# openai/Video-Pre-Training

Hardware: AMD Instinct MI355X
Metric: frames/sec (fwd) [+ bc_step.ms_per_step], 2x policy, 128x128x3 seq=128 (higher is better)
Workload: dtype bf16; 1 GPU; foundation-model-2x policy forward (IMPALA CNN + 4-layer banded transformer + heads), batch=64 seq=128 uint8 128x128x3 frames per GPU, KV memory carried, random-init weights; global_batch=64, seq_len=128, parallelism=dp1 replicas (no collective in forward; BC step: gradient all-reduce)

## Files before the change

### video-pre-training_amd/csrc/vpt_conv3x3.hip

```cpp
#include "vpt_common.h"
#include "vpt_kernels.h"
#include <stdlib.h>
#include <type_traits>
#ifndef VPT_EPI_NO_CLAMP_RELU
#define VPT_EPI_NO_CLAMP_RELU 0
#endif
#ifdef VPT_CONV_PROFILE
#define CONV_ABLATE (a.ablate)
#else
#define CONV_ABLATE 0
#endif
#if defined(VPT_CONV_PROFILE) && defined(VPT_CONV_FWD_ABLATE)
#define FWD_NO_DMA (VPT_CONV_FWD_ABLATE == 1 || VPT_CONV_FWD_ABLATE == 4)
#define FWD_NO_HALO (VPT_CONV_FWD_ABLATE == 2 || VPT_CONV_FWD_ABLATE == 4)
#else
#define FWD_NO_DMA 0
#define FWD_NO_HALO 0
#endif
#define A_RS 80
#define A_BYTES (324 * A_RS)
#define B_BYTES (3 * 128 * 64)
#define KK_OFF (A_BYTES + 2 * B_BYTES)
#define KK_BYTES (9 * 128 * 4)
#define BT_OFF (KK_OFF + KK_BYTES + 64)
#define SMEM_BYTES (BT_OFF + 512)
#define PT_RS 272
static_assert(256 * PT_RS <= KK_OFF, "the pooled mode's output tile must fit below the epilogue table");

__device__ __forceinline__ int sub_row(int i) { return ((i >> 4) ^ (i >> 2) ^ (i >> 3)) & 1; }

template <int U> __device__ __forceinline__ f32x4 ac_get(const f32x16& v) {
  return __builtin_shufflevector(v, v, 4 * U, 4 * U + 1, 4 * U + 2, 4 * U + 3);
}
template <int U> __device__ __forceinline__ void ac_set(f32x16& v, const f32x4 c) {
  const f32x16 w = __builtin_shufflevector(c, c, 0, 1, 2, 3, -1, -1, -1, -1, -1, -1, -1, -1, -1, -1, -1, -1);
  if constexpr (U == 0) v = __builtin_shufflevector(v, w, 16, 17, 18, 19, 4, 5, 6, 7, 8, 9, 10, 11, 12, 13, 14, 15);
  else if constexpr (U == 1) v = __builtin_shufflevector(v, w, 0, 1, 2, 3, 16, 17, 18, 19, 8, 9, 10, 11, 12, 13, 14, 15);
  else if constexpr (U == 2) v = __builtin_shufflevector(v, w, 0, 1, 2, 3, 4, 5, 6, 7, 16, 17, 18, 19, 12, 13, 14, 15);
  else v = __builtin_shufflevector(v, w, 0, 1, 2, 3, 4, 5, 6, 7, 8, 9, 10, 11, 16, 17, 18, 19);
}

template <bool TRACE, int MODE, int TR = 16>
__global__ __launch_bounds__(TR * 16, 2) void vpt_conv3x3_kernel(VptConv3x3Args a) {
  static_assert(TR == 16 || TR == 32, "tile rows");
  constexpr int NWAVE = TR / 4, NTHR = 64 * NWAVE;
  constexpr int HPIX = (TR + 2) * 18;
  constexpr int NA = (HPIX * 4 + NTHR - 1) / NTHR;
  constexpr int NDMA = 24 / NWAVE;
  constexpr int A_SZ = HPIX * A_RS, KK_O = A_SZ + 2 * B_BYTES, BT_O = KK_O + KK_BYTES + 64, SMEM_SZ = BT_O + 512;
  constexpr int NKK = (9 * 128 + NTHR - 1) / NTHR;
  static_assert(TR != 16 || (A_SZ == A_BYTES && KK_O == KK_OFF && SMEM_SZ <= SMEM_BYTES), "16-row layout");
  static_assert((MODE != 4 && MODE != 7) || TR == 16, "the pool-fused epilogue is written for 16 x 16 tiles");
  constexpr bool GATE = MODE == 6;
  constexpr bool PMASK = MODE == 7;
  constexpr bool PACKED_RELU = MODE == 0;
  constexpr bool CLAMP_RELU = (MODE == 1 || MODE == 5) && !VPT_EPI_NO_CLAMP_RELU;
  constexpr float RELU_S = CLAMP_RELU ? 0x1p-40f : 1.f, RELU_INV = 0x1p40f;
  constexpr bool BWD = (MODE == 2 || MODE == 3 || MODE == 6), HAS_RES = (MODE == 1 || MODE == 3 || MODE == 5), POOL = (MODE == 4 || MODE == 7), RES_AFF = MODE == 5;
  constexpr bool FWD16 = (MODE == 0 || MODE == 1 || MODE == 4 || MODE == 5 || MODE == 7);
  static_assert(FWD16 == !BWD, "forward modes: 16x16x32 loop and native-layout epilogue; dgrad modes: 32x32x16 loop and lane-swap epilogue");
  static_assert(!POOL || FWD16, "the pool-fused epilogue reads the 16x16 accumulators");
  constexpr bool DEFER_STORES = MODE != 3;
  __shared__ __attribute__((aligned(16))) unsigned char smem[SMEM_SZ];
  const int tid = threadIdx.x, lane = tid & 63;
  int cu_key = -1;
  long long t_trace[3];
  if (TRACE && (FWD16 || tid == 0)) {
    t_trace[0] = wall_clock64();
    const unsigned hw = __builtin_amdgcn_s_getreg((31 << 11) | 4);
    const unsigned xcc = __builtin_amdgcn_s_getreg((3 << 11) | 20);
    cu_key = (int)(((xcc & 15u) << 8) | ((hw >> 8) & 0xffu));
  }
  const int w = __builtin_amdgcn_readfirstlane(tid >> 6);
  const int wm = w >> 1, wn = w & 1;
  const int hi = lane >> 5, l31 = lane & 31;
  const int tilesX = a.W >> 4, tilesY = a.H / TR;
  int L = xcd_remap(blockIdx.x, gridDim.x);
  const int nt = L % a.NT; L /= a.NT;
  const int tx = L % tilesX; L /= tilesX;
  const int ty = L % tilesY;
  const int f = L / tilesY;
  const int tx0 = tx * 16, ty0 = ty * TR;
  const int NCB = a.Cin >> 5;
  const int HW = a.H * a.W;

  int a_loff[NA];
  unsigned a_gbyte[NA];
  unsigned a_inside = 0;
#pragma unroll
  for (int m = 0; m < NA; ++m) {
    const int q = tid + NTHR * m;
    const int P = FWD16 ? ((q >> 5) << 3) + 2 * (q & 3) + ((q >> 4) & 1) : ((q >> 5) << 3) + (q & 7);
    const int part = FWD16 ? 2 * ((q >> 3) & 1) + ((q >> 2) & 1) : (q >> 3) & 3;
    a_loff[m] = -1;
    a_gbyte[m] = 0u;
    if (P < HPIX) {
      const int hy = P / 18, hx = P - hy * 18;
      const int y = ty0 - 1 + hy, x = tx0 - 1 + hx;
      a_loff[m] = P * A_RS + part * 16 + (FWD16 ? 16 * (P & 1) : 0);
      if (y >= 0 && y < a.H && x >= 0 && x < a.W) {
        a_gbyte[m] = (unsigned)((y * a.W + x) * 32 + part * 8) * 2u;
        a_inside |= 1u << m;
      }
    }
  }
  const op16_t* xplane = a.x + (size_t)f * NCB * HW * 32;
  constexpr int H16_STR = (NTHR / 4) * A_RS;
  static_assert(((NA - 2) * NTHR + NTHR - 1) / 32 * 8 + 7 < HPIX, "all chunks but a thread's last are inside the halo");
  const int a_l0 = a_loff[0];
  const bool a_lastok = a_loff[NA - 1] >= 0;
  const op16_t* wbase = a.wpk + (size_t)nt * NCB * 9 * 4096 + (size_t)(w * 64 + lane) * 8;
  unsigned char* bdst = smem + A_SZ + w * 1024;

#define SB() __builtin_amdgcn_sched_barrier(0)
#define NOP_() ((void)0)
#define ISSUE_B(step_, buf_)                                                                              \
  do {                                                                                                    \
    const op16_t* wp_ = wbase + (size_t)(step_) * 12288;                                                  \
    _Pragma("unroll") for (int m_ = 0; m_ < NDMA; ++m_)                                                   \
      __builtin_amdgcn_global_load_lds((const __attribute__((address_space(1))) void*)(wp_ + m_ * (NWAVE * 512)),  \
                                       (__attribute__((address_space(3))) void*)(bdst + (buf_) * B_BYTES + m_ * (NWAVE * 1024)), \
                                       16, 0, 0);                                                         \
  } while (0)
#define GLDS(m_)                                                                                          \
  do { if ((m_) < NDMA)                                                                                   \
  __builtin_amdgcn_global_load_lds((const __attribute__((address_space(1))) void*)(wp_ + (m_) * (NWAVE * 512)),    \
                                   (__attribute__((address_space(3))) void*)(bd_ + (m_) * (NWAVE * 1024)), 16, 0, 0); } while (0)
#define XA(m_) do { if ((m_) < NA) areg[m_] = *(const u32x4*)((const char*)xplane + (cbo_ + a_gbyte[m_])); } while (0)
#define WAIT_BARRIER(n_late_)                                                                             \
  do {                                                                                                    \
    asm volatile("s_waitcnt vmcnt(" #n_late_ ") lgkmcnt(0)" ::: "memory");                                \
    __builtin_amdgcn_s_barrier();                                                                         \
    asm volatile("" ::: "memory");                                                                        \
    SB();                                                                                                 \
  } while (0)

#define WRITE_HALO()                                                                                      \
  _Pragma("unroll") for (int m_ = 0; m_ < NA; ++m_)                                                       \
    if (a_loff[m_] >= 0) *(u32x4*)(smem + a_loff[m_]) = ((a_inside >> m_) & 1u) ? areg[m_] : zero4
// ... 65 lines not shown
        if (m_ + 4 < NA && a_loff[m_ + 4] >= 0) *(u32x4*)(smem + a_loff[m_ + 4]) = ((a_inside >> (m_ + 4)) & 1u) ? areg[m_ + 4] : zero4; \
        SB(); MM(1, m_, 0); SB();                                                                         \
      }                                                                                                   \
      WAIT_BARRIER(0);                                                                                    \
      MM(1, 0, 1); FB_LD(0, 0, 0, noff_); SB();                                                           \
      MM(1, 1, 1); FA_LD(0, 0, 0, 0); SB();                                                               \
      MM(1, 2, 1); FB_LD(0, 0, 1, noff_); FA_LD(0, 0, 0, 1); SB();                                        \
      MM(1, 3, 1); FA_LD(0, 0, 0, 2); FA_LD(0, 0, 0, 3); SB();                                            \
    } else if (LAST) {                                                                                    \
      GROUP_TAIL(1);                                                                                      \
    } else {                                                                                              \
      GROUP(1, NEXT_DY, 0, noff_, NOP_(), NOP_());                                                        \
    }                                                                                                     \
  } while (0)
#define LOAD_XIN(m_)                                                                                      \
  _Pragma("unroll") for (int n2_ = 0; n2_ < 2; ++n2_)                                                     \
    _Pragma("unroll") for (int p_ = 0; p_ < 2; ++p_) xq[(m_) & 1][n2_][p_] = EPI_LD(a.xin, m_, n2_, p_)
#define ROWS_TO_PIECES(src_, dst_)                                                                        \
  _Pragma("unroll") for (int j_ = 0; j_ < 4; ++j_) {                                                      \
    const auto sw_ = __builtin_amdgcn_permlane16_swap((src_)[0][j_], (src_)[1][j_], false, false);        \
    (dst_)[0][j_] = sw_[0]; (dst_)[1][j_] = sw_[1];                                                       \
  }
#define UNSWAP(v_, e_, o_)                                                                                \
  do {                                                                                                    \
    const auto s0_ = __builtin_amdgcn_permlane32_swap((v_).x, (v_).z, false, false);                      \
    const auto s1_ = __builtin_amdgcn_permlane32_swap((v_).y, (v_).w, false, false);                      \
    (e_).x = s0_[0]; (o_).x = s0_[1]; (e_).y = s1_[0]; (o_).y = s1_[1];                                   \
  } while (0)

#define GLDS16(m_)                                                                                        \
  do { if (POOL) { if (!FWD_NO_DMA) GLDS(m_); } else if ((m_) < NDMA && !FWD_NO_DMA)                      \
  __builtin_amdgcn_raw_ptr_buffer_load_lds(wrs, (__attribute__((address_space(3))) void*)(bd_ + (m_) * (NWAVE * 1024)), 16, wvoff, \
                                           (s_ + 1) * B_BYTES + (m_) * (NWAVE * 1024), 0, 0); } while (0)
#define XA16(m_) do { if (!FWD_NO_HALO) XA(m_); } while (0)
#define HALO_WR16(m_) do { if ((m_) < NA - 1 || a_lastok) *(u32x4*)(smem + a_l0 + (m_) * H16_STR) = ((a_inside >> (m_)) & 1u) ? areg[m_] : zero4; } while (0)
#define PA(j_, dy_, dx_) fp[j_] = *(const __attribute__((address_space(3))) op16x8*)((((dx_) & 1) ? aLo : aLe) + (((j_) + (dy_)) * 18 + (dx_)) * A_RS)
#define WB(tap_, u_, boff_) fw[(u_) & 1] = *(const __attribute__((address_space(3))) op16x8*)((((u_) & 1) ? bW1 : bW0) + (boff_) + (tap_) * (128 * 64) + ((u_) >> 1) * (32 * 64))
#define M16A(j_, u_) ac_set<(u_)>(ac[j_], VPT_MFMA_16X16X32(fw[(u_) & 1], fp[j_], ac_get<(u_)>(ac[j_]), 0, 0, 0))
#define G16(MM_, u_, WLD, X)                                                                              \
  do {                                                                                                    \
    MM_(0, u_); WLD; SB();                                                                                \
    MM_(1, u_); SB();                                                                                     \
    MM_(2, u_); SB();                                                                                     \
    MM_(3, u_); X; SB();                                                                                  \
    MM_(4, u_); SB();                                                                                     \
    MM_(5, u_); SB();                                                                                     \
    MM_(6, u_); SB();                                                                                     \
    MM_(7, u_); SB();                                                                                     \
  } while (0)
#define G16R(MM_, WLD, X, ndy_, ndx_)                                                                     \
  do {                                                                                                    \
    MM_(0, 3); SB(); WLD; PA(0, ndy_, ndx_); SB();                                                              \
    MM_(1, 3); SB(); PA(1, ndy_, ndx_); SB();                                                                   \
    MM_(2, 3); SB(); PA(2, ndy_, ndx_); SB();                                                                   \
    MM_(3, 3); SB(); PA(3, ndy_, ndx_); X; SB();                                                                \
    MM_(4, 3); SB(); PA(4, ndy_, ndx_); SB();                                                                   \
    MM_(5, 3); SB(); PA(5, ndy_, ndx_); SB();                                                                   \
    MM_(6, 3); SB(); PA(6, ndy_, ndx_); SB();                                                                   \
    MM_(7, 3); SB(); PA(7, ndy_, ndx_); SB();                                                                   \
  } while (0)
#define TAP16(MM_, dy_, dx_, X0, X1, X2, X3)                                                              \
  do {                                                                                                    \
    G16(MM_, 0, WB(dx_, 1, boff_), X0);                                                                   \
    G16(MM_, 1, WB(dx_, 2, boff_), X1);                                                                   \
    G16(MM_, 2, WB(dx_, 3, boff_), X2);                                                                   \
    G16R(MM_, WB((dx_) + 1, 0, boff_), X3, dy_, (dx_) + 1);                                               \
  } while (0)
#define EPI_LD16(ptr_, j_, n2_) (*(const u32x4*)((const char*)((ptr_) + cbase[n2_]) + (voff16 + (unsigned)(j_) * gj_b)))
#define XR16(j_) do { rq16[j_][0] = EPI_LD16(resp, j_, 0); rq16[j_][1] = EPI_LD16(resp, j_, 1); } while (0)
#define XR16L(j_) do { rq16[j_][0] = *(const u32x4*)((const char*)(resp + cbase[0]) + (voff16_l + (unsigned)(j_) * gj_b)); rq16[j_][1] = *(const u32x4*)((const char*)(resp + cbase[1]) + (voff16_l + (unsigned)(j_) * gj_b)); } while (0)
#define CONV_STEP16(cb_, dy_, NEXT_DY, PRE_A, WR_A, PRE_R, LAST)                                          \
  do {                                                                                                    \
    const int s_ = (cb_) * 3 + (dy_);                                                                     \
    const int boff_ = (s_ & 1) * B_BYTES, noff_ = B_BYTES - boff_;                                        \
    const op16_t* wp_ = wbase + (size_t)(s_ + 1) * 12288;      \
    unsigned char* bd_ = bdst + noff_;                                                                    \
    const unsigned cbo_ = (unsigned)((cb_) + 1) * (unsigned)HW * 64u;                 \
    if (LAST) {                                                                                           \
      TAP16(M16A, dy_, 0, NOP_(), NOP_(), NOP_(), NOP_());                                                \
    } else {                                                                                              \
      TAP16(M16A, dy_, 0, GLDS16(0), GLDS16(1), GLDS16(2), GLDS16(3));                                          \
    }                                                                                                     \
    if (PRE_A) {                                                                                          \
      TAP16(M16A, dy_, 1, GLDS16(4), GLDS16(5), do { XA16(0); XA16(1); } while (0), XA16(2));             \
      G16(M16A, 0, WB(2, 1, boff_), do { XA16(3); XA16(4); } while (0));                                  \
      G16(M16A, 1, WB(2, 2, boff_), XA16(5));                                                             \
      G16(M16A, 2, WB(2, 3, boff_), NOP_());                                                              \
      if (NA == 6) WAIT_BARRIER(6); else WAIT_BARRIER(5);                                                 \
    } else if ((PRE_R) && HAS_RES) {                                                                      \
      TAP16(M16A, dy_, 1, GLDS16(4), GLDS16(5), XR16(0), NOP_());                                           \
      G16(M16A, 0, WB(2, 1, boff_), NOP_());                                                              \
      G16(M16A, 1, WB(2, 2, boff_), NOP_());                                                              \
      G16(M16A, 2, WB(2, 3, boff_), NOP_());                                                              \
      WAIT_BARRIER(2);                                                                                         \
    } else {                                                                                              \
      if (LAST) TAP16(M16A, dy_, 1, NOP_(), NOP_(), NOP_(), NOP_());                                      \
      else TAP16(M16A, dy_, 1, GLDS16(4), GLDS16(5), NOP_(), NOP_());                                       \
      G16(M16A, 0, WB(2, 1, boff_), NOP_());                                                              \
      G16(M16A, 1, WB(2, 2, boff_), NOP_());                                                              \
      G16(M16A, 2, WB(2, 3, boff_), NOP_());                                                              \
      WAIT_BARRIER(0);                                                                                    \
    }                                                                                                     \
    if (WR_A) {    \
      _Pragma("unroll") for (int m_ = 0; m_ < 4; ++m_) {                                                  \
        if (!FWD_NO_HALO) HALO_WR16(m_); SB();                                                            \
        if (m_ + 4 < NA && !FWD_NO_HALO) HALO_WR16(m_ + 4);                                                         \
        SB(); if (m_ == 0) M16A(0, 3); else if (m_ == 1) M16A(1, 3); else if (m_ == 2) M16A(2, 3); else M16A(3, 3); SB();                                                                        \
      }                                                                                                   \
      WAIT_BARRIER(0);                                                                                    \
      WB(0, 0, noff_); PA(0, 0, 0); PA(1, 0, 0); PA(2, 0, 0); PA(3, 0, 0); SB();                          \
      M16A(4, 3); SB(); PA(4, 0, 0); SB();                                                                      \
      M16A(5, 3); SB(); PA(5, 0, 0); SB();                                                                      \
      M16A(6, 3); SB(); PA(6, 0, 0); SB();                                                                      \
      M16A(7, 3); SB(); PA(7, 0, 0); SB();                                                                      \
    } else if (LAST) {                                                                                    \
      M16A(0, 3); M16A(1, 3); M16A(2, 3); M16A(3, 3); M16A(4, 3); M16A(5, 3); M16A(6, 3); M16A(7, 3);                                    \
    } else {                                                                                              \
      G16R(M16A, WB(0, 0, noff_), NOP_(), NEXT_DY, 0);                                                    \
    }                                                                                                     \
  } while (0)
#define EO16(j_) ((j_) == 0 ? eo_top : ((j_) == 7 ? eo_bot : 3 * 128))
#define LOAD_KK16(c_)                                                                                     \
  do {                                                                                                    \
    const float* kp_ = kk16 + EO16((c_) >> 1) + ((c_) & 1) * 32;                                          \
    kq[(c_) & 1][0] = *(const f32x4*)kp_; kq[(c_) & 1][1] = *(const f32x4*)(kp_ + 4);                     \
  } while (0)

  u32x4 areg[NA];
  const u32x4 zero4 = {0u, 0u, 0u, 0u};

  ISSUE_B(0, 0);
#pragma unroll
  for (int m = 0; m < NA; ++m) areg[m] = *(const u32x4*)((const char*)xplane + a_gbyte[m]);
  float mean = 0.f, rstd = 1.f, c0f = 0.f, c1f = 0.f;
  const float* esa = a.edge_sa;
  if (!BWD) {
    if (a.kk_frame) {
      rstd = a.rs_frame[f];
      esa = a.kk_frame + (size_t)f * 9 * a.CoutPad;
    } else {
      frame_mean_rstd(a.stats_in, f, a.inv_count_in, mean, rstd);
    }
  } else if (a.coef) {
    c0f = a.coef[2 * f];
    c1f = a.coef[2 * f + 1];
  }
  if constexpr (FWD16) {
    rstd = __builtin_bit_cast(float, __builtin_amdgcn_readfirstlane(__builtin_bit_cast(int, rstd)));
    mean = __builtin_bit_cast(float, __builtin_amdgcn_readfirstlane(__builtin_bit_cast(int, mean)));
  }
  float rgate = 1.f;
  if (GATE) {
    float mg;
    frame_mean_rstd(a.gate_stats, f, a.inv_count_gate, mg, rgate);
    c0f *= rgate;
    c1f *= rgate;
  }
  {
    float* kk = (float*)(smem + KK_O);
    float ksa[NKK], ksg[NKK];
#pragma unroll
    for (int k = 0; k < NKK; ++k) {
      const int idx = tid + NTHR * k;
      const int o = (idx >> 7) * a.CoutPad + nt * 128 + (idx & 127);
      ksa[k] = (idx < 9 * 128 && !BWD) ? esa[o] : 0.f;
      ksg[k] = (idx < 9 * 128 && !BWD) ? a.edge_sg[o] : 0.f;
    }
#pragma unroll
    for (int k = 0; k < NKK; ++k) {
      const int idx = tid + NTHR * k;
      if (idx < 9 * 128) kk[idx] = (ksa[k] - rstd * mean * ksg[k]) * RELU_S;
    }
  }
  float res_s = 1.f;
  if (RES_AFF) {
    res_s = a.res_scale[f];
    if (tid < 128) ((float*)(smem + BT_O))[tid] = (nt * 128 + tid < a.Cout) ? a.res_bias[(size_t)f * a.Cout + nt * 128 + tid] : 0.f;
  }
  if constexpr (FWD16) {
#pragma unroll
    for (int m = 0; m < NA; ++m) HALO_WR16(m);
  } else {
    WRITE_HALO();
  }
  __syncthreads();

  f32x16 acc[4][2];
  f32x16 ac[8];
  f32x16 zero16;
#pragma unroll
  for (int r = 0; r < 16; ++r) zero16[r] = 0.f;

  const unsigned char* aL = smem + ((wm * 8 + sub_row(l31)) * 18 + (l31 & 15)) * A_RS + hi * 16;
  const int bsw = (l31 >> 2) & 3;
  const unsigned char* bL0 = smem + A_SZ + (wn * 64 + l31) * 64 + (((0 + hi) ^ bsw) << 4);
  const unsigned char* bL1 = smem + A_SZ + (wn * 64 + l31) * 64 + (((2 + hi) ^ bsw) << 4);

  const int c16 = lane & 15, q16 = lane >> 4;
  const int pcol = (c16 < 4) ? 2 * c16 : ((c16 < 12) ? 2 * (c16 - 4) + 1 : 2 * (c16 - 8));
  typedef const __attribute__((address_space(3))) unsigned char* lds_cptr;
// ... 5 lines not shown

  const int CB_out = a.Cout >> 5;
  const int cb0 = nt * 4 + wn * 2;
  const bool nvalid[2] = {(cb0 + 0) < CB_out, (cb0 + 1) < CB_out};
  const unsigned gm_b = (unsigned)(2 * a.W) * 64u;
  unsigned svoff[2];
#pragma unroll
  for (int j = 0; j < 2; ++j)
    svoff[j] = (unsigned)(((ty0 + wm * 8 + sub_row((l31 & 15) + 16 * j)) * a.W + tx0 + (l31 & 15)) * 32 + 16 * (l31 >> 4) + 8 * hi) * 2u;
  size_t cbase[2];
#pragma unroll
  for (int n2 = 0; n2 < 2; ++n2) cbase[n2] = (size_t)(f * CB_out + (nvalid[n2] ? cb0 + n2 : 0)) * HW * 32;
  u32x2 rq[4][2][4];
  const unsigned nvoff = (unsigned)(((ty0 + wm * 8 + sub_row(l31)) * a.W + tx0 + (l31 & 15)) * 32 + 4 * hi) * 2u;
  const unsigned voff16 = (unsigned)(((ty0 + wm * 8) * a.W + tx0 + pcol) * 32 + 8 * q16) * 2u;
  const unsigned gj_b = (unsigned)a.W * 64u;
  u32x4 rq16[8][2];

  op16x8 fa[2][4], fb[2][2];
  const op16_t* resp = a.res;
  op16x8 fp[8], fw[2];
  const __amdgpu_buffer_rsrc_t wrs = __builtin_amdgcn_make_buffer_rsrc((void*)(a.wpk + (size_t)nt * NCB * 9 * 4096), 0, NCB * 9 * 8192, 0x00020000);
  const int wvoff = (w * 64 + lane) * 16;

  if (TRACE && (FWD16 || tid == 0)) t_trace[1] = wall_clock64();
  if constexpr (FWD16) {
    if (CONV_ABLATE != 2) {
      WB(0, 0, 0);
#pragma unroll
      for (int j = 0; j < 8; ++j) PA(j, 0, 0);
      SB();
#pragma unroll
      for (int j = 0; j < 8; ++j) ac[j] = zero16;
#pragma unroll 1
      for (int cb = 0; cb + 1 < NCB; ++cb) {
        CONV_STEP16(cb, 0, 1, true, false, false, false);
        CONV_STEP16(cb, 1, 2, false, false, false, false);
        CONV_STEP16(cb, 2, 0, false, true, false, false);
      }
      CONV_STEP16(NCB - 1, 0, 1, false, false, !TRACE, false);
      CONV_STEP16(NCB - 1, 1, 2, false, false, false, false);
      CONV_STEP16(NCB - 1, 2, 0, false, false, false, true);
    } else {
#pragma unroll
      for (int j = 0; j < 8; ++j) ac[j] = zero16;
      __syncthreads();
    }
  } else if (CONV_ABLATE != 2) {
    FB_LD(0, 0, 0, 0); FA_LD(0, 0, 0, 0); FB_LD(0, 0, 1, 0); FA_LD(0, 0, 0, 1); FA_LD(0, 0, 0, 2); FA_LD(0, 0, 0, 3);
    SB();
    if (NCB > 1) {
      CONV_STEP(0, 0, 1, true, false, false, false, true);
      CONV_STEP(0, 1, 2, false, false, false, false, false);
      CONV_STEP(0, 2, 0, false, true, false, false, false);
    } else {
#pragma unroll
      for (int m = 0; m < 4; ++m)
#pragma unroll
        for (int n = 0; n < 2; ++n)
#pragma unroll
          for (int r = 0; r < 16; ++r) acc[m][n][r] = 0.f;
    }
    for (int cb = 1; cb + 1 < NCB; ++cb) {
      CONV_STEP(cb, 0, 1, true, false, false, false, false);
      CONV_STEP(cb, 1, 2, false, false, false, false, false);
      CONV_STEP(cb, 2, 0, false, true, false, false, false);
    }
    CONV_STEP(NCB - 1, 0, 1, false, false, true, false, false);
    CONV_STEP(NCB - 1, 1, 2, false, false, false, false, false);
    CONV_STEP(NCB - 1, 2, 0, false, false, false, true, false);
  } else {
#pragma unroll
    for (int m = 0; m < 4; ++m)
#pragma unroll
// ... 100 lines not shown
    }
  }
  if (DEFER_STORES)
#pragma unroll
  for (int m = 0; m < 4; ++m)
#pragma unroll
    for (int n2 = 0; n2 < NV; ++n2) {
#pragma unroll
      for (int p = 0; p < 2; ++p)
        *(u32x4*)((char*)(a.y + cbase[n2]) + (svoff[p] + (unsigned)m * gm_b)) = outv[m][n2][p];
    }
  };
  int lane_l = lane;
  asm volatile("" : "+v"(lane_l));
  const int c16_l = lane_l & 15, q16_l = lane_l >> 4;
  const int pcol_l = (c16_l < 4) ? 2 * c16_l : ((c16_l < 12) ? 2 * (c16_l - 4) + 1 : 2 * (c16_l - 8));
  const unsigned voff16_l = (unsigned)(((ty0 + wm * 8) * a.W + tx0 + pcol_l) * 32 + 8 * q16_l) * 2u;
  const int x16_ = tx0 + pcol_l;
  const int ex16 = (x16_ == 0) ? 0 : ((x16_ == a.W - 1) ? 2 : 1);
  const int eo_top = (ty0 + wm * 8 == 0) ? 0 : 3 * 128, eo_bot = (ty0 + wm * 8 + 7 == a.H - 1) ? 6 * 128 : 3 * 128;
  const float* kk16 = (const float*)(smem + KK_O) + ex16 * 128 + wn * 64 + 8 * q16_l;
  auto epilogue16 = [&](auto nv_) __attribute__((always_inline)) {
    constexpr int NV = decltype(nv_)::value;
    u32x4 outv[8][2];
    f32x4 kq[2][2];
    LOAD_KK16(0);
    SB();
    const f32x2 zero2 = {0.f, 0.f};
    const f32x2 rstd2 = {rstd * RELU_S, rstd * RELU_S}, ress2 = {res_s, res_s};
    const f32x2 relu_inv2 = {RELU_INV, RELU_INV};
    const float* btab = (const float*)(smem + BT_O) + wn * 64 + 8 * q16_l;
#pragma unroll
    for (int j = 0; j < 8; ++j) {
      if (HAS_RES && j == 0) XR16L(1);
      if (HAS_RES && j < 6) XR16L(j + 2);
      SB();
#pragma unroll
      for (int n2 = 0; n2 < 2; ++n2) {
        if (2 * j + n2 < 15) { LOAD_KK16(2 * j + n2 + 1); SB(); }
        if (n2 >= NV) continue;
        f32x4 bq[2];
        if (RES_AFF) {
          bq[0] = *(const f32x4*)(btab + n2 * 32); bq[1] = *(const f32x4*)(btab + n2 * 32 + 4);
          SB();
        }
        u32x2 pk[2];
#pragma unroll
        for (int h = 0; h < 2; ++h) {
          f32x2 v01 = {ac[j][8 * n2 + 4 * h + 0], ac[j][8 * n2 + 4 * h + 1]}, v23 = {ac[j][8 * n2 + 4 * h + 2], ac[j][8 * n2 + 4 * h + 3]};
          const f32x4 k4 = kq[n2][h];
          const f32x2 k01 = {k4.x, k4.y}, k23 = {k4.z, k4.w};
          if (PACKED_RELU) {
            v01 = rstd2 * v01 + k01;
            v23 = rstd2 * v23 + k23;
          } else if (CLAMP_RELU) {
            v01 = pk_fma_clamp01(rstd2, v01, k01);
            v23 = pk_fma_clamp01(rstd2, v23, k23);
          } else {
            v01 = __builtin_elementwise_max(rstd2 * v01 + k01, zero2);
            v23 = __builtin_elementwise_max(rstd2 * v23 + k23, zero2);
          }
          if (HAS_RES) {
            const uint32_t ra = h ? rq16[j][n2].z : rq16[j][n2].x, rb = h ? rq16[j][n2].w : rq16[j][n2].y;
            const f32x2 r01 = {op16_lo_to_f32(ra), op16_hi_to_f32(ra)}, r23 = {op16_lo_to_f32(rb), op16_hi_to_f32(rb)};
            if (RES_AFF) {
              const f32x4 b4 = bq[h];
              const f32x2 b01 = {b4.x, b4.y}, b23 = {b4.z, b4.w};
              if (CLAMP_RELU) {
                v01 = ress2 * r01 + __builtin_elementwise_fma(v01, relu_inv2, b01);
                v23 = ress2 * r23 + __builtin_elementwise_fma(v23, relu_inv2, b23);
              } else {
                v01 = ress2 * r01 + (v01 + b01);
// ... 184 lines not shown
    static_assert(BWD, "the 32x32 epilogue is written for the dgrad modes only");
    if (nvalid[1]) epilogue(std::integral_constant<int, 2>{});
    else if (nvalid[0]) epilogue(std::integral_constant<int, 1>{});
  }
#undef SB
#undef NOP_
#undef ISSUE_B
#undef GLDS
#undef XA
#undef WAIT_BARRIER
#undef WRITE_HALO
#undef MM
#undef MMZ
#undef FA_LD
#undef FB_LD
#undef GROUP_
#undef GROUP
#undef GROUP_Z
#undef GROUP_TAIL
#undef EPI_LD
#undef EPI_LDN
#undef LOAD_RES
#undef XR
#undef CONV_STEP
#undef LOAD_XIN
#undef ROWS_TO_PIECES
#undef UNSWAP
#undef HALO_WR16
#undef PA
#undef WB
#undef M16A
#undef G16
#undef G16R
#undef TAP16
#undef EPI_LD16
#undef XR16
#undef XR16L
#undef CONV_STEP16
#undef EO16
#undef LOAD_KK16
  float s_sum = s_sum2.x + s_sum2.y, s_sq = s_sq2.x + s_sq2.y;
  if (GATE) {
    float* red = (float*)(smem + KK_O + KK_BYTES);
    s_sum = wave_sum(s_sum + s_sq);
    if (lane == 0) red[w] = s_sum;
    __syncthreads();
    if (tid == 0) atomicAdd(a.gate_u + f, (double)((red[0] + red[1]) + (red[2] + red[3])));
  }
  if (!BWD && a.stats_out) {
    float* red = (float*)(smem + KK_O + KK_BYTES);
    s_sum = wave_sum(s_sum);
    s_sq = wave_sum(s_sq);
    if (lane == 0) { red[w] = s_sum; red[NWAVE + w] = s_sq; }
    __syncthreads();
    if (tid == 0) {
      float t1 = (red[0] + red[1]) + (red[2] + red[3]), t2 = (red[NWAVE] + red[NWAVE + 1]) + (red[NWAVE + 2] + red[NWAVE + 3]);
      if (NWAVE == 8) {
        t1 += (red[4] + red[5]) + (red[6] + red[7]);
        t2 += (red[12] + red[13]) + (red[14] + red[15]);
      }
      atomicAdd(a.stats_out + 2 * f, (double)t1);
      atomicAdd(a.stats_out + 2 * f + 1, (double)t2);
    }
  }
  if (TRACE && tid == 0) {
    long long* t = a.trace + (size_t)blockIdx.x * 12;
    t[0] = t_trace[0]; t[1] = t_trace[1]; t[2] = t_trace[2]; t[3] = wall_clock64(); t[4] = cu_key; t[5] = 0;
    for (int k = 0; k < 5; ++k) t[6 + k] = 0;
  }
}

#define S_W_BYTES (9 * 32 * 64)
#define S_NBUF 3
#define S_KK_OFF (S_NBUF * (A_BYTES + S_W_BYTES))
#define S_BYTES (S_KK_OFF + 9 * 32 * 4 + 64)

template <bool HAS_RES>
__global__ __launch_bounds__(512, 1) void vpt_conv3x3_small_kernel(VptConv3x3Args a) {
  __shared__ __attribute__((aligned(16))) unsigned char smem[S_BYTES];
  const int tid = threadIdx.x, lane = tid & 63;
  const int w = __builtin_amdgcn_readfirstlane(tid >> 6);
  const int hi = lane >> 5, l31 = lane & 31;
  const int tilesX = a.W >> 4, tilesY = a.H >> 4;
  const int CB_out = a.Cout >> 5;
  int L = blockIdx.x;
  const int cbo = L % CB_out; L /= CB_out;
  const int tx = L % tilesX; L /= tilesX;
  const int ty = L % tilesY;
  const int f = L / tilesY;
  const int nt = cbo >> 2, qo = cbo & 3;
  const int tx0 = tx * 16, ty0 = ty * 16;
  const int NCB = a.Cin >> 5;
  const int HW = a.H * a.W;

  int a_loff[3];
  unsigned a_gbyte[3];
  unsigned a_inside = 0;
#pragma unroll
  for (int m = 0; m < 3; ++m) {
    const int q = tid + 512 * m;
    const int P = ((q >> 5) << 3) + (q & 7), part = (q >> 3) & 3;
// ... 147 lines not shown
extern "C" void vpt_conv3x3_set_trace(void* buf) { g_conv_trace = (long long*)buf; }

extern "C" int vpt_conv3x3_launch(const VptConv3x3Args* a_in, hipStream_t stream) {
  int ablate = 0, extra_lds = 0;
#ifdef VPT_CONV_PROFILE
  static int ablate_env = -1, extra_lds_env = 0;
  if (ablate_env < 0) {
    const char* e = getenv("VPT_CONV_ABLATE");
    ablate_env = e ? atoi(e) : 0;
    const char* xl = getenv("VPT_CONV_EXTRA_LDS");
    extra_lds_env = xl ? atoi(xl) : 0;
    if (extra_lds_env > 0) {
      (void)hipFuncSetAttribute((const void*)vpt_conv3x3_kernel<false, 0>, hipFuncAttributeMaxDynamicSharedMemorySize, extra_lds_env);
      (void)hipFuncSetAttribute((const void*)vpt_conv3x3_kernel<false, 1>, hipFuncAttributeMaxDynamicSharedMemorySize, extra_lds_env);
    }
  }
  ablate = ablate_env; extra_lds = extra_lds_env;
#endif
  VptConv3x3Args a_copy = *a_in;
  a_copy.ablate = ablate;
  a_copy.trace = g_conv_trace;
  const VptConv3x3Args* a = &a_copy;
  if ((a->H & 15) || (a->W & 15) || (a->Cin & 31) || (a->Cout & 31) || a->frames <= 0) return -1;
  const long grid = (long)a->frames * (a->H >> 4) * (a->W >> 4) * a->NT;
  if (grid > 0x7fffffffL) return -2;
  const int mode = a->bwd ? (a->res ? 3 : (a->gate_stats ? 6 : 2)) : (a->pool ? (a->pool_mask ? 7 : 4) : (a->res ? (a->res_bias ? 5 : 1) : 0));
  if (a->pool_mask && !a->pool) return -1;
  if (a->gate_stats && (!a->bwd || a->res || !a->gate_u || a->trace)) return -1;
  if ((a->res_bias != nullptr) != (a->res_scale != nullptr) || (a->res_bias && (a->bwd || !a->res))) return -1;
  if ((a->kk_frame != nullptr) != (a->rs_frame != nullptr) || (a->kk_frame && a->bwd)) return -1;
  if (a->bwd && (!a->xin || !a->coef)) return -1;
  if (a->pool && (a->bwd || a->res || (a->tiling != 1 && a->tiling != 3) || a->trace || !a->seam_r || !a->seam_c)) return -1;
  if (!a->bwd && a->tiling != 1 && a->tiling != 2 && a->tiling != 3) return -1;
  if (!a->bwd && !a->trace && a->tiling == 2) {
    const long sgrid = (long)a->frames * (a->H >> 4) * (a->W >> 4) * (a->Cout >> 5);
    if (a->res) hipLaunchKernelGGL((vpt_conv3x3_small_kernel<true>), dim3((unsigned)sgrid), dim3(512), 0, stream, *a);
    else hipLaunchKernelGGL((vpt_conv3x3_small_kernel<false>), dim3((unsigned)sgrid), dim3(512), 0, stream, *a);
    return hipGetLastError() == hipSuccess ? 0 : -3;
  }
#define LAUNCH_(T_, M_) hipLaunchKernelGGL((vpt_conv3x3_kernel<T_, M_>), dim3((unsigned)grid), dim3(256), extra_lds, stream, *a)
  if (a->trace && mode > 3) return -1;
  if (mode == 6) { LAUNCH_(false, 6); return hipGetLastError() == hipSuccess ? 0 : -3; }
  if (mode == 7) { LAUNCH_(false, 7); return hipGetLastError() == hipSuccess ? 0 : -3; }
  if (!a->trace && !a->bwd && mode != 4 && (a->H & 31) == 0 && a->tiling == 3 && !extra_lds) {
    const long g32 = grid >> 1;
#define LAUNCH32_(M_) hipLaunchKernelGGL((vpt_conv3x3_kernel<false, M_, 32>), dim3((unsigned)g32), dim3(512), 0, stream, *a)
    if (mode == 0) LAUNCH32_(0); else if (mode == 1) LAUNCH32_(1); else LAUNCH32_(5);
#undef LAUNCH32_
    return hipGetLastError() == hipSuccess ? 0 : -3;
  }
  if (a->trace) { if (mode == 0) LAUNCH_(true, 0); else if (mode == 1) LAUNCH_(true, 1); else if (mode == 2) LAUNCH_(true, 2); else LAUNCH_(true, 3); }
  else { if (mode == 0) LAUNCH_(false, 0); else if (mode == 1) LAUNCH_(false, 1); else if (mode == 2) LAUNCH_(false, 2); else if (mode == 3) LAUNCH_(false, 3); else if (mode == 4) LAUNCH_(false, 4); else LAUNCH_(false, 5); }
#undef LAUNCH_
  return hipGetLastError() == hipSuccess ? 0 : -3;
}

template <bool MASK>
__global__ __launch_bounds__(256) void vpt_pool_seam_kernel(VptPoolSeamArgs a) {
  typedef short i16x8 __attribute__((ext_vector_type(8)));
  __shared__ float red[4][4][18];
  const int tid = threadIdx.x, lane = tid & 63, w = tid >> 6;
  const int PH = a.H >> 1, PW = a.W >> 1, TY = a.H >> 4, TX = a.W >> 4;
  const int n_row = (TY - 1) * PW;
  const int col_len = PH - (TY - 1);
  const int n_pix = n_row + (TX - 1) * col_len;
  const int cb = blockIdx.x % a.CB, f = blockIdx.x / a.CB;
// ... 113 lines not shown
```

Before: 81210 frames/s.

## Use buffer loads for halo and overlap halo LDS writes with last-tap MFMAs

In the FWD16 conv path, halo loads now use raw buffer loads with an out-of-range offset sentinel, so hardware bounds checking returns zeros and the per-chunk inside/outside select is dropped. The halo LDS writes move earlier, interleaved with the MFMAs of the third weight-slice group after a new barrier that ensures the old halo is no longer being read. This lets the writes overlap compute instead of sitting in a separate serialized block. It adds an extra workgroup barrier per step and a size guard for the 32-bit buffer range.

```diff
diff --git a/video-pre-training_amd/csrc/vpt_conv3x3.hip b/video-pre-training_amd/csrc/vpt_conv3x3.hip
--- a/video-pre-training_amd/csrc/vpt_conv3x3.hip
+++ b/video-pre-training_amd/csrc/vpt_conv3x3.hip
@@ -13,10 +13,13 @@
 #if defined(VPT_CONV_PROFILE) && defined(VPT_CONV_FWD_ABLATE)
 #define FWD_NO_DMA (VPT_CONV_FWD_ABLATE == 1 || VPT_CONV_FWD_ABLATE == 4)
 #define FWD_NO_HALO (VPT_CONV_FWD_ABLATE == 2 || VPT_CONV_FWD_ABLATE == 4)
+#define FWD_NO_HALO_BAR (VPT_CONV_FWD_ABLATE == 8)
 #else
 #define FWD_NO_DMA 0
 #define FWD_NO_HALO 0
+#define FWD_NO_HALO_BAR 0
 #endif
+#define HALO_OOB 0x80000000u
 #define A_RS 80
 #define A_BYTES (324 * A_RS)
 #define B_BYTES (3 * 128 * 64)
@@ -93,7 +96,7 @@
     const int P = FWD16 ? ((q >> 5) << 3) + 2 * (q & 3) + ((q >> 4) & 1) : ((q >> 5) << 3) + (q & 7);
     const int part = FWD16 ? 2 * ((q >> 3) & 1) + ((q >> 2) & 1) : (q >> 3) & 3;
     a_loff[m] = -1;
-    a_gbyte[m] = 0u;
+    a_gbyte[m] = FWD16 ? HALO_OOB : 0u;
     if (P < HPIX) {
       const int hy = P / 18, hx = P - hy * 18;
       const int y = ty0 - 1 + hy, x = tx0 - 1 + hx;
@@ -105,6 +108,7 @@
     }
   }
   const op16_t* xplane = a.x + (size_t)f * NCB * HW * 32;
+  const __amdgpu_buffer_rsrc_t xrs = __builtin_amdgcn_make_buffer_rsrc((void*)xplane, 0, NCB * HW * 64, 0x00020000);
   constexpr int H16_STR = (NTHR / 4) * A_RS;
   static_assert(((NA - 2) * NTHR + NTHR - 1) / 32 * 8 + 7 < HPIX, "all chunks but a thread's last are inside the halo");
   const int a_l0 = a_loff[0];
@@ -236,8 +240,9 @@
   do { if (POOL) { if (!FWD_NO_DMA) GLDS(m_); } else if ((m_) < NDMA && !FWD_NO_DMA)                      \
   __builtin_amdgcn_raw_ptr_buffer_load_lds(wrs, (__attribute__((address_space(3))) void*)(bd_ + (m_) * (NWAVE * 1024)), 16, wvoff, \
                                            (s_ + 1) * B_BYTES + (m_) * (NWAVE * 1024), 0, 0); } while (0)
-#define XA16(m_) do { if (!FWD_NO_HALO) XA(m_); } while (0)
-#define HALO_WR16(m_) do { if ((m_) < NA - 1 || a_lastok) *(u32x4*)(smem + a_l0 + (m_) * H16_STR) = ((a_inside >> (m_)) & 1u) ? areg[m_] : zero4; } while (0)
+#define XA16_(m_, soff_) do { if ((m_) < NA) areg[m_] = __builtin_bit_cast(u32x4, __builtin_amdgcn_raw_buffer_load_b128(xrs, (int)a_gbyte[m_], (int)(soff_), 0)); } while (0)
+#define XA16(m_) do { if (!FWD_NO_HALO) XA16_(m_, cbo_); } while (0)
+#define HALO_WR16(m_) do { if ((m_) < NA && ((m_) < NA - 1 || a_lastok)) *(u32x4*)(smem + a_l0 + (m_) * H16_STR) = areg[m_]; } while (0)
 #define PA(j_, dy_, dx_) fp[j_] = *(const __attribute__((address_space(3))) op16x8*)((((dx_) & 1) ? aLo : aLe) + (((j_) + (dy_)) * 18 + (dx_)) * A_RS)
 #define WB(tap_, u_, boff_) fw[(u_) & 1] = *(const __attribute__((address_space(3))) op16x8*)((((u_) & 1) ? bW1 : bW0) + (boff_) + (tap_) * (128 * 64) + ((u_) >> 1) * (32 * 64))
 #define M16A(j_, u_) ac_set<(u_)>(ac[j_], VPT_MFMA_16X16X32(fw[(u_) & 1], fp[j_], ac_get<(u_)>(ac[j_]), 0, 0, 0))
@@ -263,6 +268,25 @@
     MM_(6, 3); SB(); PA(6, ndy_, ndx_); SB();                                                                   \
     MM_(7, 3); SB(); PA(7, ndy_, ndx_); SB();                                                                   \
   } while (0)
+#define G16H(MM_, u_, WLD, W1, W2, W3, W4, W5, W6)                                                        \
+  do {                                                                                                    \
+    MM_(0, u_); WLD; SB();                                                                                \
+    MM_(1, u_); W1; SB();                                                                                 \
+    MM_(2, u_); W2; SB();                                                                                 \
+    MM_(3, u_); W3; SB();                                                                                 \
+    MM_(4, u_); W4; SB();                                                                                 \
+    MM_(5, u_); W5; SB();                                                                                 \
+    MM_(6, u_); W6; SB();                                                                                 \
+    MM_(7, u_); SB();                                                                                     \
+  } while (0)
+#define HALO_DEAD_BARRIER()                                                                               \
+  do {                                                                                                    \
+    asm volatile("s_waitcnt lgkmcnt(0)" ::: "memory");                                                    \
+    __builtin_amdgcn_s_barrier();                                                                         \
+    asm volatile("" ::: "memory");                                                                        \
+    SB();                                                                                                 \
+  } while (0)
+#define HALO_SW16(m_) do { if (!FWD_NO_HALO) HALO_WR16(m_); } while (0)
 #define TAP16(MM_, dy_, dx_, X0, X1, X2, X3)                                                              \
   do {                                                                                                    \
     G16(MM_, 0, WB(dx_, 1, boff_), X0);                                                                   \
@@ -297,6 +321,13 @@
       G16(M16A, 1, WB(2, 2, boff_), NOP_());                                                              \
       G16(M16A, 2, WB(2, 3, boff_), NOP_());                                                              \
       WAIT_BARRIER(2);                                                                                         \
+    } else if (WR_A) {    \
+      TAP16(M16A, dy_, 1, GLDS16(4), GLDS16(5), NOP_(), NOP_());                                          \
+      G16(M16A, 0, WB(2, 1, boff_), NOP_());                                                              \
+      G16(M16A, 1, WB(2, 2, boff_), NOP_());                                                              \
+      if (!FWD_NO_HALO_BAR) HALO_DEAD_BARRIER();    \
+      G16H(M16A, 2, WB(2, 3, boff_), HALO_SW16(0), HALO_SW16(1), HALO_SW16(2), HALO_SW16(3), HALO_SW16(4), HALO_SW16(5)); \
+      WAIT_BARRIER(0);                \
     } else {                                                                                              \
       if (LAST) TAP16(M16A, dy_, 1, NOP_(), NOP_(), NOP_(), NOP_());                                      \
       else TAP16(M16A, dy_, 1, GLDS16(4), GLDS16(5), NOP_(), NOP_());                                       \
@@ -305,19 +336,7 @@
       G16(M16A, 2, WB(2, 3, boff_), NOP_());                                                              \
       WAIT_BARRIER(0);                                                                                    \
     }                                                                                                     \
-    if (WR_A) {    \
-      _Pragma("unroll") for (int m_ = 0; m_ < 4; ++m_) {                                                  \
-        if (!FWD_NO_HALO) HALO_WR16(m_); SB();                                                            \
-        if (m_ + 4 < NA && !FWD_NO_HALO) HALO_WR16(m_ + 4);                                                         \
-        SB(); if (m_ == 0) M16A(0, 3); else if (m_ == 1) M16A(1, 3); else if (m_ == 2) M16A(2, 3); else M16A(3, 3); SB();                                                                        \
-      }                                                                                                   \
-      WAIT_BARRIER(0);                                                                                    \
-      WB(0, 0, noff_); PA(0, 0, 0); PA(1, 0, 0); PA(2, 0, 0); PA(3, 0, 0); SB();                          \
-      M16A(4, 3); SB(); PA(4, 0, 0); SB();                                                                      \
-      M16A(5, 3); SB(); PA(5, 0, 0); SB();                                                                      \
-      M16A(6, 3); SB(); PA(6, 0, 0); SB();                                                                      \
-      M16A(7, 3); SB(); PA(7, 0, 0); SB();                                                                      \
-    } else if (LAST) {                                                                                    \
+    if (LAST) {                                                                                           \
       M16A(0, 3); M16A(1, 3); M16A(2, 3); M16A(3, 3); M16A(4, 3); M16A(5, 3); M16A(6, 3); M16A(7, 3);                                    \
     } else {                                                                                              \
       G16R(M16A, WB(0, 0, noff_), NOP_(), NEXT_DY, 0);                                                    \
@@ -334,8 +353,13 @@
   const u32x4 zero4 = {0u, 0u, 0u, 0u};
 
   ISSUE_B(0, 0);
-#pragma unroll
-  for (int m = 0; m < NA; ++m) areg[m] = *(const u32x4*)((const char*)xplane + a_gbyte[m]);
+  if constexpr (FWD16) {
+#pragma unroll
+    for (int m = 0; m < NA; ++m) XA16_(m, 0);
+  } else {
+#pragma unroll
+    for (int m = 0; m < NA; ++m) areg[m] = *(const u32x4*)((const char*)xplane + a_gbyte[m]);
+  }
   float mean = 0.f, rstd = 1.f, c0f = 0.f, c1f = 0.f;
   const float* esa = a.edge_sa;
   if (!BWD) {
@@ -871,6 +895,9 @@
 #undef M16A
 #undef G16
 #undef G16R
+#undef G16H
+#undef HALO_DEAD_BARRIER
+#undef HALO_SW16
 #undef TAP16
 #undef EPI_LD16
 #undef XR16
@@ -1119,6 +1146,7 @@
   if (a->bwd && (!a->xin || !a->coef)) return -1;
   if (a->pool && (a->bwd || a->res || (a->tiling != 1 && a->tiling != 3) || a->trace || !a->seam_r || !a->seam_c)) return -1;
   if (!a->bwd && a->tiling != 1 && a->tiling != 2 && a->tiling != 3) return -1;
+  if (!a->bwd && a->tiling != 2 && (long)a->Cin * a->H * a->W * 2 > (1L << 30)) return -2;
   if (!a->bwd && !a->trace && a->tiling == 2) {
     const long sgrid = (long)a->frames * (a->H >> 4) * (a->W >> 4) * (a->Cout >> 5);
     if (a->res) hipLaunchKernelGGL((vpt_conv3x3_small_kernel<true>), dim3((unsigned)sgrid), dim3(512), 0, stream, *a);
```

Measured after the change: 81780 frames/s, median of 6. No clear change (+0.7%).

## Prefetch residual tiles into LDS via buffer DMA during last conv step

Applied to the files above, without the earlier changes.

For forward 16-row tiles with a residual input, the last conv K-step now issues buffer_load_lds DMA of several residual rows into the free B-operand buffer. The epilogue then reads those rows from LDS instead of global memory, and some epilogue-table loads are skipped for those rows. The aim is to hide residual-load latency behind the final MFMA step and shorten the epilogue's global-load stall. It also adds profiling-only trace timers and a fixed-halo ablation path. The LDS reuse depends on buffer-parity assumptions, and the conditional skipping of LOAD_KK16 needs to line up with which registers are actually consumed.

```diff
diff --git a/video-pre-training_amd/csrc/vpt_conv3x3.hip b/video-pre-training_amd/csrc/vpt_conv3x3.hip
--- a/video-pre-training_amd/csrc/vpt_conv3x3.hip
+++ b/video-pre-training_amd/csrc/vpt_conv3x3.hip
@@ -13,9 +13,11 @@
 #if defined(VPT_CONV_PROFILE) && defined(VPT_CONV_FWD_ABLATE)
 #define FWD_NO_DMA (VPT_CONV_FWD_ABLATE == 1 || VPT_CONV_FWD_ABLATE == 4)
 #define FWD_NO_HALO (VPT_CONV_FWD_ABLATE == 2 || VPT_CONV_FWD_ABLATE == 4)
+#define FWD_FIXED_HALO (VPT_CONV_FWD_ABLATE == 8)
 #else
 #define FWD_NO_DMA 0
 #define FWD_NO_HALO 0
+#define FWD_FIXED_HALO 0
 #endif
 #define A_RS 80
 #define A_BYTES (324 * A_RS)
@@ -60,6 +62,7 @@
   constexpr bool FWD16 = (MODE == 0 || MODE == 1 || MODE == 4 || MODE == 5 || MODE == 7);
   static_assert(FWD16 == !BWD, "forward modes: 16x16x32 loop and native-layout epilogue; dgrad modes: 32x32x16 loop and lane-swap epilogue");
   static_assert(!POOL || FWD16, "the pool-fused epilogue reads the 16x16 accumulators");
+  constexpr bool RES_LDS = FWD16 && HAS_RES && TR == 16;
   constexpr bool DEFER_STORES = MODE != 3;
   __shared__ __attribute__((aligned(16))) unsigned char smem[SMEM_SZ];
   const int tid = threadIdx.x, lane = tid & 63;
@@ -273,6 +276,11 @@
 #define EPI_LD16(ptr_, j_, n2_) (*(const u32x4*)((const char*)((ptr_) + cbase[n2_]) + (voff16 + (unsigned)(j_) * gj_b)))
 #define XR16(j_) do { rq16[j_][0] = EPI_LD16(resp, j_, 0); rq16[j_][1] = EPI_LD16(resp, j_, 1); } while (0)
 #define XR16L(j_) do { rq16[j_][0] = *(const u32x4*)((const char*)(resp + cbase[0]) + (voff16_l + (unsigned)(j_) * gj_b)); rq16[j_][1] = *(const u32x4*)((const char*)(resp + cbase[1]) + (voff16_l + (unsigned)(j_) * gj_b)); } while (0)
+#define RDMA16(p_)                                                                                        \
+  do { if constexpr (RES_LDS)                                                                             \
+  __builtin_amdgcn_raw_ptr_buffer_load_lds(((p_) & 1) ? rrs1 : rrs0, (__attribute__((address_space(3))) void*)(bd_ + (p_) * (NWAVE * 1024)), 16, (int)voff16, \
+                                           (int)((unsigned)(1 + ((p_) >> 1)) * gj_b), 0, 0); } while (0)
+#define XRL16(j_) do { rq16[j_][0] = *(const __attribute__((address_space(3))) u32x4*)(rl16 + (2 * (j_) - 2) * (NWAVE * 1024)); rq16[j_][1] = *(const __attribute__((address_space(3))) u32x4*)(rl16 + (2 * (j_) - 1) * (NWAVE * 1024)); } while (0)
 #define CONV_STEP16(cb_, dy_, NEXT_DY, PRE_A, WR_A, PRE_R, LAST)                                          \
   do {                                                                                                    \
     const int s_ = (cb_) * 3 + (dy_);                                                                     \
@@ -281,11 +289,11 @@
     unsigned char* bd_ = bdst + noff_;                                                                    \
     const unsigned cbo_ = (unsigned)((cb_) + 1) * (unsigned)HW * 64u;                 \
     if (LAST) {                                                                                           \
-      TAP16(M16A, dy_, 0, NOP_(), NOP_(), NOP_(), NOP_());                                                \
+      TAP16(M16A, dy_, 0, RDMA16(0), RDMA16(1), RDMA16(2), RDMA16(3));                                    \
     } else {                                                                                              \
       TAP16(M16A, dy_, 0, GLDS16(0), GLDS16(1), GLDS16(2), GLDS16(3));                                          \
     }                                                                                                     \
-    if (PRE_A) {                                                                                          \
+    if (PRE_A) {                                                                                       \
       TAP16(M16A, dy_, 1, GLDS16(4), GLDS16(5), do { XA16(0); XA16(1); } while (0), XA16(2));             \
       G16(M16A, 0, WB(2, 1, boff_), do { XA16(3); XA16(4); } while (0));                                  \
       G16(M16A, 1, WB(2, 2, boff_), XA16(5));                                                             \
@@ -298,7 +306,7 @@
       G16(M16A, 2, WB(2, 3, boff_), NOP_());                                                              \
       WAIT_BARRIER(2);                                                                                         \
     } else {                                                                                              \
-      if (LAST) TAP16(M16A, dy_, 1, NOP_(), NOP_(), NOP_(), NOP_());                                      \
+      if (LAST) TAP16(M16A, dy_, 1, RDMA16(4), RDMA16(5), NOP_(), NOP_());                                \
       else TAP16(M16A, dy_, 1, GLDS16(4), GLDS16(5), NOP_(), NOP_());                                       \
       G16(M16A, 0, WB(2, 1, boff_), NOP_());                                                              \
       G16(M16A, 1, WB(2, 2, boff_), NOP_());                                                              \
@@ -335,7 +343,18 @@
 
   ISSUE_B(0, 0);
 #pragma unroll
-  for (int m = 0; m < NA; ++m) areg[m] = *(const u32x4*)((const char*)xplane + a_gbyte[m]);
+  for (int m = 0; m < NA; ++m) {
+    if (FWD16 && FWD_FIXED_HALO) {
+      const int q = tid + NTHR * m;
+      const int P = ((q >> 5) << 3) + 2 * (q & 3) + ((q >> 4) & 1), part = 2 * ((q >> 3) & 1) + ((q >> 2) & 1);
+      const int hy = P / 18, hx = P - hy * 18;
+      const bool in0 = P < HPIX && hy >= 1 && hx >= 1 && hy - 1 < a.H && hx - 1 < a.W;
+      areg[m] = *(const u32x4*)((const char*)a.x + (in0 ? (unsigned)(((hy - 1) * a.W + hx - 1) * 32 + part * 8) * 2u : 0u));
+    } else {
+      areg[m] = *(const u32x4*)((const char*)xplane + a_gbyte[m]);
+    }
+  }
+  int d_trace[2] = {0, 0};
   float mean = 0.f, rstd = 1.f, c0f = 0.f, c1f = 0.f;
   const float* esa = a.edge_sa;
   if (!BWD) {
@@ -370,6 +389,13 @@
       ksa[k] = (idx < 9 * 128 && !BWD) ? esa[o] : 0.f;
       ksg[k] = (idx < 9 * 128 && !BWD) ? a.edge_sg[o] : 0.f;
     }
+    if (TRACE && FWD16) {
+      SB();
+      d_trace[0] = (int)(wall_clock64() - t_trace[0]);
+      asm volatile("s_waitcnt vmcnt(0)" ::: "memory");
+      d_trace[1] = (int)(wall_clock64() - t_trace[0]);
+      SB();
+    }
 #pragma unroll
     for (int k = 0; k < NKK; ++k) {
       const int idx = tid + NTHR * k;
@@ -441,6 +467,7 @@
       SB();
 #pragma unroll
       for (int j = 0; j < 8; ++j) ac[j] = zero16;
+      __amdgpu_buffer_rsrc_t rrs0 = wrs, rrs1 = wrs;
 #pragma unroll 1
       for (int cb = 0; cb + 1 < NCB; ++cb) {
         CONV_STEP16(cb, 0, 1, true, false, false, false);
@@ -449,6 +476,11 @@
       }
       CONV_STEP16(NCB - 1, 0, 1, false, false, !TRACE, false);
       CONV_STEP16(NCB - 1, 1, 2, false, false, false, false);
+      if constexpr (RES_LDS) {
+        const unsigned plane_b = (unsigned)HW * 64u;
+        rrs0 = __builtin_amdgcn_make_buffer_rsrc((void*)(resp + cbase[0]), 0, nvalid[0] ? plane_b : 0u, 0x00020000);
+        rrs1 = __builtin_amdgcn_make_buffer_rsrc((void*)(resp + cbase[1]), 0, nvalid[1] ? plane_b : 0u, 0x00020000);
+      }
       CONV_STEP16(NCB - 1, 2, 0, false, false, false, true);
     } else {
 #pragma unroll
@@ -615,12 +647,18 @@
     const float* btab = (const float*)(smem + BT_O) + wn * 64 + 8 * q16_l;
 #pragma unroll
     for (int j = 0; j < 8; ++j) {
-      if (HAS_RES && j == 0) XR16L(1);
-      if (HAS_RES && j < 6) XR16L(j + 2);
+      if constexpr (RES_LDS) {
+        lds_cptr rl16 = (lds_cptr)smem + A_SZ + ((NCB & 1) ? B_BYTES : 0) + w * 1024 + lane_l * 16;
+        if (j < 3) XRL16(j + 1);
+        if (j < 4) XR16L(j + 4);
+      } else {
+        if (HAS_RES && j == 0) XR16L(1);
+        if (HAS_RES && j < 6) XR16L(j + 2);
+      }
       SB();
 #pragma unroll
       for (int n2 = 0; n2 < 2; ++n2) {
-        if (2 * j + n2 < 15) { LOAD_KK16(2 * j + n2 + 1); SB(); }
+        if (2 * j + n2 < 15) { if (!RES_LDS || ((2 * j + n2 + 1) >> 1) < 2 || ((2 * j + n2 + 1) >> 1) == 7) LOAD_KK16(2 * j + n2 + 1); SB(); }
         if (n2 >= NV) continue;
         f32x4 bq[2];
         if (RES_AFF) {
@@ -875,6 +913,8 @@
 #undef EPI_LD16
 #undef XR16
 #undef XR16L
+#undef RDMA16
+#undef XRL16
 #undef CONV_STEP16
 #undef EO16
 #undef LOAD_KK16
@@ -905,7 +945,8 @@
   if (TRACE && tid == 0) {
     long long* t = a.trace + (size_t)blockIdx.x * 12;
     t[0] = t_trace[0]; t[1] = t_trace[1]; t[2] = t_trace[2]; t[3] = wall_clock64(); t[4] = cu_key; t[5] = 0;
-    for (int k = 0; k < 5; ++k) t[6 + k] = 0;
+    t[6] = d_trace[0]; t[7] = d_trace[1];
+    for (int k = 2; k < 5; ++k) t[6 + k] = 0;
   }
 }
 
```

Result: no change. 79300 frames/s before, 79520 frames/s after (median of 6 runs) (+0.3%).
